# smoltcp-rs/smoltcp

Hardware: AMD Instinct MI355X
Metric: GiB/s checksummed (device-resident), batched 1500B segments, 1/2/4/8 GPU (higher is better)
Workload: dtype u8; 1 GPU; C2: 1048576 x 1500 B IPv4/UDP datagrams, fixed stride, emit (tx) + verify (rx, 1/64 single-bit corrupted); records_per_gpu=1048576, parallelism=shard x1 (no collective)

## Files before the change

### include/smolcsum_tools.h

```cpp
#ifndef SMOLCSUM_TOOLS_H
#define SMOLCSUM_TOOLS_H

#include "smolcsum.h"

#ifdef __cplusplus
extern "C" {
#endif

enum {
    SMOL_SYNTH_UDP4 = 0,
    SMOL_SYNTH_TCP4 = 1,
    SMOL_SYNTH_V6MIX = 2,
    SMOL_SYNTH_ETH_TCP4 = 3,
    SMOL_SYNTH_RANDOM = 4
};

int smol_csum_tool_synth(smol_csum_ctx_t* ctx, uint8_t* d_buf, const smol_csum_batch_t* batch,
                         int profile, uint64_t seed, void* stream);

int smol_csum_tool_corrupt(smol_csum_ctx_t* ctx, uint8_t* d_buf, const smol_csum_batch_t* batch,
                           uint32_t every, uint64_t seed, void* stream);

int smol_csum_tool_set_shape(smol_csum_ctx_t* ctx, int shape);

int smol_csum_tool_set_variant(smol_csum_ctx_t* ctx, int variant);

int smol_csum_tool_set_tile(smol_csum_ctx_t* ctx, int records);

int smol_csum_tool_set_max_blocks(smol_csum_ctx_t* ctx, uint32_t max_blocks);

int smol_csum_tool_set_xcd_remap(smol_csum_ctx_t* ctx, int on);

int smol_csum_tool_set_launch_records(smol_csum_ctx_t* ctx, uint64_t records);

int smol_csum_tool_set_fields_kernel(smol_csum_ctx_t* ctx, int kernel);

int smol_csum_tool_set_vcopy_stores(smol_csum_ctx_t* ctx, int nt);

int smol_csum_tool_stream_read(smol_csum_ctx_t* ctx, const uint8_t* d_buf, uint64_t bytes,
                               uint32_t* d_sink, void* stream);

int smol_csum_tool_field_probe(smol_csum_ctx_t* ctx, uint8_t* d_buf, uint64_t bytes, uint64_t stride,
                               uint32_t f1, uint32_t f2, void* stream);
int smol_csum_tool_field_probe_list(smol_csum_ctx_t* ctx, uint8_t* d_buf, uint64_t bytes, const uint64_t* d_addrs,
                                    const uint32_t* d_piece_first, int flags, void* stream);
int smol_csum_tool_segment_probe(smol_csum_ctx_t* ctx, uint8_t* d_buf, uint64_t bytes, const uint32_t* d_bitmap, int flags,
                                 void* stream);
int smol_csum_tool_field_scatter(smol_csum_ctx_t* ctx, uint8_t* d_buf, uint64_t bytes, const uint64_t* d_addrs,
                                 const uint16_t* d_vals, uint64_t n, int flags, void* stream);
int smol_csum_tool_auto_shape(uint32_t len, int has_desc);

int smol_csum_tool_pick(int variant, int shape, int desc_staged, int op, const smol_csum_batch_t* batch, int nhc,
                        int out[3]);
int smol_csum_tool_variant_info(int variant, int out[4]);
int smol_csum_tool_form(int variant, int op, int out[13]);
int smol_csum_tool_walk_launch(int variant, int op, int implicit, int nhc, int shape, int out[4]);

const char* smol_csum_tool_kernel_for(const smol_csum_ctx_t* ctx, int op, const smol_csum_batch_t* batch);
const char* smol_csum_tool_kernel_name(const smol_csum_ctx_t* ctx, int op, int has_desc);

uint32_t smol_csum_tool_last_launch(void);

int smol_csum_tool_variant_built(int variant);

#ifdef __cplusplus
}
#endif

#endif
```

### smoltcp_amd/_lib.py

```python
from __future__ import annotations

import ctypes
import os

_HERE = os.path.dirname(os.path.abspath(__file__))
LIB_PATH = os.environ.get("SMOLCSUM_LIB") or os.path.join(_HERE, "libsmolcsum.so")
EXP_LIB_PATH = os.path.join(_HERE, "libsmolcsum_exp.so")

SMOL_OK, SMOL_EINVAL, SMOL_ENODEV, SMOL_EHIP, SMOL_ERANGE, SMOL_ENOMEM = 0, -1, -2, -3, -4, -5
ERROR_NAMES = {
    SMOL_EINVAL: "SMOL_EINVAL",
    SMOL_ENODEV: "SMOL_ENODEV",
    SMOL_EHIP: "SMOL_EHIP",
    SMOL_ERANGE: "SMOL_ERANGE",
    SMOL_ENOMEM: "SMOL_ENOMEM",
}

ABI_SYMBOLS = [
    "smol_csum_data", "smol_csum_combine", "smol_csum_pseudo_header_v4",
    "smol_csum_pseudo_header_v6", "smol_csum_pseudo_header", "smol_csum_ctx_create",
    "smol_csum_ctx_destroy", "smol_csum_batch_data", "smol_csum_batch_emit",
    "smol_csum_batch_verify", "smol_csum_batch_copy_emit", "smol_csum_batch_emit_fields",
    "smol_csum_batch_verify_copy",
    "smol_csum_apply_fields", "smol_csum_batch_emit_frag",
    "smol_csum_batch_verify_frag", "smol_csum_batch_verify_reassemble", "smol_csum_batch_fragment_emit",
    "smol_csum_batch_nhc_udp_emit",
    "smol_csum_batch_nhc_udp_verify", "smol_csum_last_error", "smol_csum_abi_version",
]
TOOL_SYMBOLS = [
    "smol_csum_tool_synth", "smol_csum_tool_corrupt", "smol_csum_tool_set_shape",
    "smol_csum_tool_set_variant", "smol_csum_tool_set_tile",
    "smol_csum_tool_set_max_blocks", "smol_csum_tool_auto_shape", "smol_csum_tool_stream_read",
    "smol_csum_tool_set_xcd_remap", "smol_csum_tool_set_launch_records",
    "smol_csum_tool_field_probe",
    "smol_csum_tool_field_probe_list", "smol_csum_tool_segment_probe", "smol_csum_tool_field_scatter",
    "smol_csum_tool_variant_built",
    "smol_csum_tool_kernel_name", "smol_csum_tool_kernel_for", "smol_csum_tool_last_launch",
    "smol_csum_tool_pick", "smol_csum_tool_variant_info", "smol_csum_tool_form",
    "smol_csum_tool_set_fields_kernel", "smol_csum_tool_walk_launch", "smol_csum_tool_set_vcopy_stores",
]
OPTIONAL_TOOL_SYMBOLS = ("smol_csum_tool_variant_built", "smol_csum_tool_kernel_for", "smol_csum_tool_segment_probe",
                         "smol_csum_tool_pick", "smol_csum_tool_variant_info", "smol_csum_tool_form",
                         "smol_csum_tool_set_fields_kernel", "smol_csum_tool_walk_launch",
                         "smol_csum_tool_set_vcopy_stores")


class SmolError(RuntimeError):
    def __init__(self, rc: int, what: str, detail: str = ""):
        name = ERROR_NAMES.get(rc, str(rc))
        super().__init__(f"{what} failed: {name}" + (f" ({detail})" if detail else ""))
        self.rc = rc


class Caps(ctypes.Structure):

    _fields_ = [
        ("ipv4", ctypes.c_uint8),
        ("udp", ctypes.c_uint8),
        ("tcp", ctypes.c_uint8),
        ("icmpv4", ctypes.c_uint8),
        ("icmpv6", ctypes.c_uint8),
        ("reserved", ctypes.c_uint8 * 3),
    ]


class BatchC(ctypes.Structure):

    _fields_ = [
        ("desc", ctypes.c_void_p),
        ("n", ctypes.c_uint64),
        ("stride", ctypes.c_uint64),
        ("len", ctypes.c_uint32),
        ("kind", ctypes.c_uint8),
        ("flags", ctypes.c_uint8),
        ("reserved", ctypes.c_uint8 * 2),
    ]

# ... 137 lines not shown
    L.smol_csum_tool_set_variant.restype = i32
    L.smol_csum_tool_set_tile.argtypes = [vp, i32]
    L.smol_csum_tool_set_tile.restype = i32
    L.smol_csum_tool_set_max_blocks.argtypes = [vp, u32]
    L.smol_csum_tool_set_max_blocks.restype = i32
    L.smol_csum_tool_set_xcd_remap.argtypes = [vp, ctypes.c_int]
    L.smol_csum_tool_set_xcd_remap.restype = i32
    L.smol_csum_tool_set_launch_records.argtypes = [vp, u64]
    L.smol_csum_tool_set_launch_records.restype = i32
    L.smol_csum_tool_stream_read.argtypes = [vp, vp, u64, vp, vp]
    L.smol_csum_tool_stream_read.restype = i32
    L.smol_csum_tool_field_probe.argtypes = [vp, vp, u64, u64, ctypes.c_uint32, ctypes.c_uint32, vp]
    L.smol_csum_tool_field_probe.restype = i32
    L.smol_csum_tool_field_probe_list.argtypes = [vp, vp, u64, vp, vp, ctypes.c_int, vp]
    L.smol_csum_tool_field_probe_list.restype = i32
    L.smol_csum_tool_field_scatter.argtypes = [vp, vp, u64, vp, vp, u64, ctypes.c_int, vp]
    L.smol_csum_tool_field_scatter.restype = i32
    L.smol_csum_tool_auto_shape.argtypes = [u32, i32]
    L.smol_csum_tool_auto_shape.restype = i32
    L.smol_csum_tool_kernel_name.argtypes = [vp, i32, i32]
    L.smol_csum_tool_kernel_name.restype = ctypes.c_char_p
    L.smol_csum_tool_last_launch.argtypes = []
    L.smol_csum_tool_last_launch.restype = u32
    optional = {
        "smol_csum_tool_variant_built": ([i32], i32),
        "smol_csum_tool_segment_probe": ([vp, vp, u64, vp, ctypes.c_int, vp], i32),
        "smol_csum_tool_kernel_for": ([vp, i32, vp], ctypes.c_char_p),
        "smol_csum_tool_pick": ([i32, i32, i32, i32, ctypes.POINTER(BatchC), i32, ctypes.POINTER(i32)], i32),
        "smol_csum_tool_variant_info": ([i32, ctypes.POINTER(i32)], i32),
        "smol_csum_tool_form": ([i32, i32, ctypes.POINTER(i32)], i32),
        "smol_csum_tool_set_fields_kernel": ([vp, i32], i32),
        "smol_csum_tool_walk_launch": ([i32, i32, i32, i32, i32, ctypes.POINTER(i32)], i32),
        "smol_csum_tool_set_vcopy_stores": ([vp, i32], i32),
    }
    assert set(optional) == set(OPTIONAL_TOOL_SYMBOLS)
    for name in OPTIONAL_TOOL_SYMBOLS:
        if hasattr(L, name):
            f = getattr(L, name)
            f.argtypes, f.restype = optional[name]
    _LIBS[path] = L
    return L


def check(rc: int, what: str, L: ctypes.CDLL | None = None) -> None:
    if rc != SMOL_OK:
        detail = (L or lib()).smol_csum_last_error().decode(errors="replace") if rc == SMOL_EHIP else ""
        raise SmolError(rc, what, detail)
```

### smoltcp_amd/csrc/csum_api.cpp

```cpp
#include <hip/hip_runtime.h>

#include <cstdint>
#include <cstring>
#include <new>
#include <string>

#include "../../include/smolcsum.h"
#include "../../include/smolcsum_tools.h"
#include "csum_dispatch.h"

using namespace smolcsum;

struct smol_csum_ctx {
    int device;
    int num_cu;
    uint32_t max_blocks;
    int shape;
    int variant;
    uint8_t* dummy;
    int tile_records;
    bool max_blocks_set;
    int xcd_remap;
    uint64_t launch_records;
    uint64_t* stage;
    uint32_t* stage_flags;
    void* stage_stream;
    bool stage_recorded;
    hipEvent_t stage_done;
    uint32_t* sample_host;
    hipEvent_t sample_ev;
    bool sample_pending;
    int desc_staged;
    uint32_t since_probe;
    int fields_kernel;
    bool vcopy_nt;
};

namespace {
constexpr uint32_t kSample = 256;
constexpr uint32_t kReprobe = 64;
}

namespace smolcsum {

uint32_t resident_blocks(const void* kernel, uint32_t num_cu, uint32_t max_blocks) {
    if (num_cu == 0) return max_blocks;
    int per_cu = 0;
    if (hipOccupancyMaxActiveBlocksPerMultiprocessor(&per_cu, kernel, 256, 0) != hipSuccess || per_cu < 1)
        per_cu = 1;
    const uint64_t cap = (uint64_t)per_cu * num_cu;
    return (uint32_t)(cap < max_blocks ? cap : max_blocks);
}

}

namespace {

thread_local std::string g_last_error;

int hip_fail(hipError_t e, const char* what) {
    g_last_error = std::string(what) + ": " + hipGetErrorString(e);
// ... 87 lines not shown
hipError_t for_launches(const smol_csum_ctx_t* ctx, const smol_csum_batch_t* b, const KParams& p, F&& launch) {
    const uint64_t per = ctx->launch_records && ctx->launch_records < b->n ? ctx->launch_records : b->n;
    for (uint64_t i0 = 0; i0 < b->n; i0 += per) {
        KParams q = p;
        q.n = b->n - i0 < per ? b->n - i0 : per;
        if (b->desc) q.desc = b->desc + i0;
        else q.buf = p.buf + i0 * b->stride;
        const hipError_t e = launch(i0, q);
        if (e != hipSuccess) return e;
    }
    return hipSuccess;
}

PickCtx pick_ctx(const smol_csum_ctx_t* ctx) { return {ctx->variant, ctx->shape, ctx->desc_staged}; }

const char* family_kernel(int family) {
    switch (family) {
        case F_TILE: case F_STRIPE: return "csum_tile_kernel";
        case F_XWALK: return "xwalk_kernel";
        case F_DWALK: return "dwalk_kernel";
        case F_COPY: return "copy_kernel";
        case F_XCOPY: return "xcopy_kernel";
        default: return "csum_kernel";
    }
}

bool has_desc_auto(const smol_csum_ctx_t* ctx, const smol_csum_batch_t* b, const uint8_t* d_addrs) {
    return b->desc && !d_addrs && ctx->variant < 0 && !(b->flags & SMOL_BATCH_FIELD_STORES);
}

bool capturing(hipStream_t s) {
    hipStreamCaptureStatus st = hipStreamCaptureStatusNone;
    return hipStreamIsCapturing(s, &st) == hipSuccess && st != hipStreamCaptureStatusNone;
}

void update_desc_choice(smol_csum_ctx_t* ctx, hipStream_t s) {
    if (capturing(s)) return;
    if (ctx->sample_pending && hipEventQuery(ctx->sample_ev) == hipSuccess) {
        ctx->sample_pending = false;
        uint32_t n = ctx->sample_host[kSample], staged = 0;
        for (uint32_t i = 0; i < n && i < kSample; ++i) staged += ctx->sample_host[i] != 0u;
        ctx->desc_staged = n == 0 || 2 * staged >= n ? 1 : 0;
        ctx->since_probe = 0;
    }
    if (!ctx->desc_staged && !ctx->sample_pending && ++ctx->since_probe >= kReprobe) ctx->desc_staged = 1;
}

void sample_desc_choice(smol_csum_ctx_t* ctx, uint64_t n, hipStream_t s) {
    if (capturing(s) || ctx->sample_pending) return;
    const uint32_t waves = (uint32_t)((n + 7) / 8 < kSample ? (n + 7) / 8 : kSample);
    ctx->sample_host[kSample] = waves;
    if (hipMemcpyAsync(ctx->sample_host, ctx->stage_flags, waves * sizeof(uint32_t), hipMemcpyDeviceToHost, s) !=
            hipSuccess ||
        hipEventRecord(ctx->sample_ev, s) != hipSuccess) {
        (void)hipGetLastError();
        return;
    }
    ctx->sample_pending = true;
}

int run(smol_csum_ctx_t* ctx, int mode, uint8_t* d_buf, const smol_csum_batch_t* b,
        const smol_checksum_caps_t* caps, uint16_t* d_out, uint8_t* d_status, void* stream,
        const uint8_t* d_src = nullptr, const smol_csum_copy_t* d_copy = nullptr,
        const uint8_t* d_addrs = nullptr) {
    KParams p = base_params(ctx, d_buf, b, caps);
    p.src = d_src;
    p.copy = d_copy;
    if (d_addrs) p.kind = KIND_NHC_UDP;
    p.addrs = d_addrs;
    p.out16 = d_out;
    p.status = d_status;
    p.num_cu = ctx->max_blocks_set ? 0u : cu_count(ctx);
    p.xcd_remap = ctx->xcd_remap >= 0 ? (uint32_t)ctx->xcd_remap : (uint32_t)xcd_remap_auto(mode, b);
    DeviceGuard guard(ctx->device);
    if (!guard.ok) return hip_fail(hipErrorInvalidDevice, "hipSetDevice");
    const hipStream_t s = (hipStream_t)stream;
    const uint64_t per = ctx->launch_records ? ctx->launch_records : b->n;
    if (per < b->n) {
        for (uint64_t i0 = 0; i0 < b->n; i0 += per) {
            smol_csum_batch_t sub = *b;
            sub.n = b->n - i0 < per ? b->n - i0 : per;
            uint8_t* buf = d_buf;
            if (b->desc) sub.desc = b->desc + i0;
            else buf = d_buf + i0 * b->stride;
            const uint64_t keep = ctx->launch_records;
            ctx->launch_records = 0;
            const int rc = run(ctx, mode, buf, &sub, caps, d_out ? d_out + i0 : nullptr, d_status ? d_status + i0 : nullptr,
                               stream, d_src, d_copy ? d_copy + i0 : nullptr, d_addrs ? d_addrs + 32 * i0 : nullptr);
            ctx->launch_records = keep;
            if (rc != SMOL_OK) return rc;
        }
        return SMOL_OK;
    }
    const bool desc_auto = mode == MODE_EMIT && has_desc_auto(ctx, b, d_addrs);
    if (desc_auto) update_desc_choice(ctx, s);
    const Pick k = pick_kernel(pick_ctx(ctx), mode, b, p);
    if (mode == MODE_EMIT && variant_is(k.variant, V_STAGED)) {
        if (ctx->stage_recorded && ctx->stage_stream != stream) {
            hipError_t ew = hipStreamWaitEvent(s, ctx->stage_done, 0);
            if (ew != hipSuccess) return hip_fail(ew, "hipStreamWaitEvent (staged emit)");
        }
        for (uint64_t i0 = 0; i0 < b->n; i0 += kStageChunk) {
            KParams q = p;
            q.n = b->n - i0 < kStageChunk ? b->n - i0 : kStageChunk;
            if (b->desc) q.desc = b->desc + i0;
            else q.buf = d_buf + i0 * b->stride;
            if (d_status) q.status = d_status + i0;
            q.stage = ctx->stage;
            q.stage_flags = ctx->stage_flags;
            const hipError_t e = k.family == F_DWALK ? launch_dwalk(mode, k.variant, q, s) : launch_xwalk(mode, k.variant, q, s);
            if (e != hipSuccess) return hip_fail(e, "checksum kernel launch");
        }
        if (desc_auto) sample_desc_choice(ctx, b->n < kStageChunk ? b->n : kStageChunk, s);
        hipError_t er = hipEventRecord(ctx->stage_done, s);
        if (er != hipSuccess) return hip_fail(er, "hipEventRecord (staged emit)");
        ctx->stage_stream = stream;
        ctx->stage_recorded = true;
        return SMOL_OK;
    }
    hipError_t e = hipSuccess;
    switch (k.family) {
        case F_XCOPY: e = launch_xcopy(k.variant, p, s); break;
        case F_DWALK: e = launch_dwalk(mode, k.variant, p, s); break;
        case F_XWALK: e = launch_xwalk(mode, k.variant, p, s); break;
        case F_STRIPE: e = launch_stripe(mode, p, s); break;
        case F_TILE:
            e = launch_tile(mode, k.shape, find_variant(k.variant)->tile_loads, ctx->tile_records, p, ctx->max_blocks, s);
            break;
        default: e = launch_csum(mode, k.shape, k.variant, p, ctx->max_blocks, s); break;
    }
    if (e != hipSuccess) return hip_fail(e, mode == MODE_COPY ? "copy-emit kernel launch" : "checksum kernel launch");
    return SMOL_OK;
}

}

extern "C" {



int smol_csum_ctx_create(int device, smol_csum_ctx_t** out) {
    if (!out) return SMOL_EINVAL;
    *out = nullptr;
    int count = 0;
    if (hipGetDeviceCount(&count) != hipSuccess || count <= 0) {
        g_last_error = "no HIP device";
        return SMOL_ENODEV;
    }
    if (device < 0 || device >= count) return SMOL_ENODEV;
// ... 11 lines not shown
        return hip_fail(e, "hipMemset");
    }
    uint64_t* stage = nullptr;
    uint32_t* flags = nullptr;
    hipEvent_t done = nullptr;
    e = hipMalloc(&stage, kStageChunk * sizeof(uint64_t));
    if (e == hipSuccess) e = hipMalloc(&flags, (kStageChunk / 8 + 64) * sizeof(uint32_t));
    if (e == hipSuccess) e = hipEventCreateWithFlags(&done, hipEventDisableTiming);
    uint32_t* sample = nullptr;
    hipEvent_t sev = nullptr;
    if (e == hipSuccess) e = hipHostMalloc(&sample, (kSample + 1) * sizeof(uint32_t), hipHostMallocDefault);
    if (e == hipSuccess) e = hipEventCreateWithFlags(&sev, hipEventDisableTiming);
    if (e != hipSuccess) {
        (void)hipFree(dummy);
        if (stage) (void)hipFree(stage);
        if (flags) (void)hipFree(flags);
        if (sample) (void)hipHostFree(sample);
        return hip_fail(e, "context allocation");
    }
    auto* c = new (std::nothrow) smol_csum_ctx;
    if (!c) {
        (void)hipFree(dummy);
        (void)hipFree(stage);
        (void)hipFree(flags);
        (void)hipEventDestroy(done);
        (void)hipHostFree(sample);
        (void)hipEventDestroy(sev);
        return SMOL_ENOMEM;
    }
    c->dummy = dummy;
    c->stage = stage;
    c->stage_flags = flags;
    c->stage_stream = nullptr;
    c->stage_recorded = false;
    c->stage_done = done;
    c->sample_host = sample;
    c->sample_ev = sev;
    c->sample_pending = false;
    c->desc_staged = 1;
    c->since_probe = 0;
    c->fields_kernel = FK_AUTO;
    c->vcopy_nt = false;
    c->tile_records = 32;
    c->max_blocks_set = false;
    c->xcd_remap = -1;
    c->launch_records = 0;
    c->device = device;
    c->num_cu = cus;
    c->max_blocks = kNaturalGrid;
    c->shape = -1;
    c->variant = -1;
    *out = c;
    return SMOL_OK;
}

int smol_csum_ctx_destroy(smol_csum_ctx_t* ctx) {
    if (!ctx) return SMOL_OK;
    {
        DeviceGuard guard(ctx->device);
        (void)hipFree(ctx->dummy);
        (void)hipFree(ctx->stage);
        (void)hipFree(ctx->stage_flags);
        (void)hipEventDestroy(ctx->stage_done);
        if (ctx->sample_pending) (void)hipEventSynchronize(ctx->sample_ev);
        (void)hipHostFree(ctx->sample_host);
        (void)hipEventDestroy(ctx->sample_ev);
    }
// ... 186 lines not shown
    if (!ctx || !variant_built(variant)) return SMOL_EINVAL;
    ctx->variant = variant;
    return SMOL_OK;
}

int smol_csum_tool_set_tile(smol_csum_ctx_t* ctx, int records) {
    if (!ctx || (records != 32 && records != 64)) return SMOL_EINVAL;
    ctx->tile_records = records;
    return SMOL_OK;
}

int smol_csum_tool_set_max_blocks(smol_csum_ctx_t* ctx, uint32_t max_blocks) {
    if (!ctx) return SMOL_EINVAL;
    ctx->max_blocks = max_blocks ? max_blocks : kNaturalGrid;
    ctx->max_blocks_set = max_blocks != 0;
    return SMOL_OK;
}

int smol_csum_tool_set_xcd_remap(smol_csum_ctx_t* ctx, int on) {
    if (!ctx || on < -1) return SMOL_EINVAL;
    ctx->xcd_remap = on;
    return SMOL_OK;
}

int smol_csum_tool_set_launch_records(smol_csum_ctx_t* ctx, uint64_t records) {
    if (!ctx) return SMOL_EINVAL;
    ctx->launch_records = records;
    return SMOL_OK;
}

int smol_csum_tool_set_fields_kernel(smol_csum_ctx_t* ctx, int kernel) {
    if (!ctx || kernel < FK_AUTO || kernel > FK_DWALK) return SMOL_EINVAL;
    ctx->fields_kernel = kernel;
    return SMOL_OK;
}

int smol_csum_tool_set_vcopy_stores(smol_csum_ctx_t* ctx, int nt) {
    if (!ctx || (nt != 0 && nt != 1)) return SMOL_EINVAL;
    ctx->vcopy_nt = nt == 1;
    return SMOL_OK;
}

int smol_csum_tool_stream_read(smol_csum_ctx_t* ctx, const uint8_t* d_buf, uint64_t bytes,
                               uint32_t* d_sink, void* stream) {
    if (!ctx || !d_buf || !d_sink || (bytes & 15u) || ((uintptr_t)d_buf & 15u)) return SMOL_EINVAL;
    return on_device(ctx, "stream-read kernel launch", [&] {
        return launch_stream_read(d_buf, bytes, d_sink, cu_count(ctx) * 8u, (hipStream_t)stream);
    });
}

int smol_csum_tool_field_probe(smol_csum_ctx_t* ctx, uint8_t* d_buf, uint64_t bytes, uint64_t stride,
                               uint32_t f1, uint32_t f2, void* stream) {
    if (!ctx || !d_buf || (bytes & 15u) || ((uintptr_t)d_buf & 15u) || stride == 0 || f1 == ~0u) return SMOL_EINVAL;
    return on_device(ctx, "field-probe kernel launch", [&] {
        return launch_field_probe(d_buf, bytes, stride, f1, f2, cu_count(ctx) * 8u, (hipStream_t)stream);
    });
}

int smol_csum_tool_field_probe_list(smol_csum_ctx_t* ctx, uint8_t* d_buf, uint64_t bytes, const uint64_t* d_addrs,
                                    const uint32_t* d_piece_first, int flags, void* stream) {
    if (!ctx || !d_buf || !d_addrs || !d_piece_first || (bytes & 15u) || ((uintptr_t)d_buf & 15u) || (flags & ~1))
        return SMOL_EINVAL;
    return on_device(ctx, "field-probe kernel launch", [&] {
        return launch_field_probe_list(d_buf, bytes, d_addrs, d_piece_first, flags & 1, cu_count(ctx) * 8u, (hipStream_t)stream);
    });
}
// ... 124 lines not shown
```

### smoltcp_amd/csrc/csum_launch.h

```cpp
#pragma once

#include <hip/hip_runtime.h>
#include <stdint.h>

#include <atomic>

#include "../../include/smolcsum.h"
#include "csum_variants.h"

namespace smolcsum {

enum { MODE_DATA = 0, MODE_EMIT = 1, MODE_VERIFY = 2, MODE_COPY = 3 };
static_assert(MODE_DATA == kOpData && MODE_EMIT == kOpEmit && MODE_VERIFY == kOpVerify && MODE_COPY == kOpCopy, "csum_variants.h");

constexpr uint32_t KIND_NHC_UDP = 0x10;
constexpr uint32_t KIND_IPHDR_ONLY = 0x200;
__host__ __device__ __forceinline__ uint32_t desc_kind(uint32_t w) {
    return (w & 0xffu) | (((w >> 8) & SMOL_REC_IPHDR_ONLY) ? KIND_IPHDR_ONLY : 0u);
}

enum {
    CFG_G8U6 = 0,
    CFG_G16U3 = 1,
    CFG_G16U6 = 2,
// ... 163 lines not shown
inline void note_launch(uint32_t kern, uint32_t var, uint32_t g, uint32_t u) {
    g_last_launch.store(kern << 24 | (var & 0xffu) << 16 | (g & 0xffu) << 8 | (u & 0xffu),
                        std::memory_order_relaxed);
}

constexpr uint64_t kMaxGridBlocks = 0xFFFFFFull;
__host__ __device__ inline uint32_t grid_blocks(uint64_t want, uint64_t cap) {
    uint64_t b = want < cap ? want : cap;
    b = b < kMaxGridBlocks ? b : kMaxGridBlocks;
    return (uint32_t)(b ? b : 1);
}

uint32_t resident_blocks(const void* kernel, uint32_t num_cu, uint32_t max_blocks);

hipError_t launch_csum(int mode, int shape, int var, const KParams& p, uint32_t max_blocks, hipStream_t s);
template <int MODE, bool IMPLICIT>
hipError_t launch_walk(int shape, int var, const KParams& p, uint32_t max_blocks, hipStream_t s);
template <int MODE, bool IMPLICIT>
hipError_t launch_walk_nhc(int shape, int var, const KParams& p, uint32_t max_blocks, hipStream_t s);
hipError_t launch_tile(int mode, int shape, int var, int tile_records, const KParams& p, uint32_t max_blocks,
                       hipStream_t s);

hipError_t launch_stripe(int mode, const KParams& p, hipStream_t s);
hipError_t launch_dwalk(int mode, int variant, const KParams& p, hipStream_t s);
hipError_t launch_xcopy(int variant, const KParams& p, hipStream_t s);
hipError_t launch_copy_kernel(int shape, int var, const KParams& p, uint32_t max_blocks, hipStream_t s);
hipError_t launch_xwalk(int mode, int variant, const KParams& p, hipStream_t s);
constexpr uint64_t kStageChunk = 1ull << 21;
hipError_t launch_seg_pass(const KParams& p, hipStream_t s, int form = 0);
template <bool IMPLICIT>
hipError_t launch_walk_fields(int shape, const KParams& p, uint32_t max_blocks, hipStream_t s);
hipError_t launch_xwalk_fields(const KParams& p, hipStream_t s);
hipError_t launch_dwalk_fields(const KParams& p, hipStream_t s);

struct VCopyArgs {
    uint8_t* dst;
    const smol_csum_slot_t* slots;
    smol_csum_span_t* spans;
};
hipError_t launch_vcopy(int shape, bool nt, const KParams& p, const VCopyArgs& v, uint32_t max_blocks,
                        hipStream_t s);

struct SynthParams {
    uint8_t* buf;
    const smol_csum_desc_t* desc;
    uint64_t n;
    uint64_t stride;
    uint32_t len;
    uint32_t profile;
    uint64_t seed;
};
hipError_t launch_synth(const SynthParams& p, uint32_t max_blocks, hipStream_t s);
hipError_t launch_corrupt(const SynthParams& p, uint32_t every, hipStream_t s);
hipError_t launch_frag(int mode, const KParams& p, const smol_csum_frag_group_t* groups, uint64_t ngroups,
                       hipStream_t s);
struct FragCopyArgs {
    uint8_t* dst;
    const smol_csum_slot_t* slots;
    smol_csum_dgram_t* dgrams;
};
hipError_t launch_fragcopy(const KParams& p, const smol_csum_frag_group_t* groups, uint64_t ngroups,
                           const FragCopyArgs& v, hipStream_t s);
struct FragCutArgs {
    uint8_t* dst;
    const smol_csum_fragplan_t* plans;
    uint32_t frame_stride;
// ... 16 lines not shown
```

### smoltcp_amd/csrc/csum_xwalk.hip

```cpp
#include "csum_dispatch.h"
#include "csum_walk.h"

namespace smolcsum {

namespace xwalk {

constexpr int WIN_CH = 16;
constexpr int WAVES = 4;


}

template <int MODE, int R, class F>
__global__ __launch_bounds__(64 * F::WV) __attribute__((amdgpu_waves_per_eu(F::WPE > 0 ? F::WPE : 1))) void xwalk_kernel(KParams p) {
    using namespace xwalk;
    constexpr bool NOSTORE = F::NOSTORE, SEG = F::SEG, PERSIST = F::PERSIST, HALF = F::HALF, STAGE = F::STAGE;
    constexpr int NTS = F::NTS, HINT = F::HINT, WV = F::WV, STEPS = F::STEPS;
    constexpr bool EMIT = MODE == MODE_EMIT;
    constexpr int G = 64 / R;
    constexpr int NS = 16 / R;
    constexpr int GPB = WV * R;
    __shared__ u32x4 win[GPB][WIN_CH];
    __shared__ uint32_t spanbuf[GPB];
    const int wl = (int)(threadIdx.x & 63);
// ... 205 lines not shown
            if (mine && lane == 0 && r % 8 == 0) p.stage_flags[r / 8] = 1u;
        } else {
            if (wsA != ~0ull && lane < 8) seg_store(wsA + 8u * (uint32_t)lane);
            if (wsB != ~0ull && lane < 8) seg_store(wsB + 8u * (uint32_t)lane);
        }
    } else {
        if (mine)
            finish_gates<G, MODE, false, decltype(rd), 0, false, NOSTORE, (NTS & 128) != 0, false, EMIT && F::FIELDS>(
                p, g, lane == 0 ? tot : 0u, rd, winb, hd, a0, r, lane);
    }
    if (!more) break;
    wave_lds_sync();
    tw = tn;
    ++step;
    }
}

template <int MODE, int R, class F>
static void launch_xwalk_form(uint32_t blocks, const KParams& p, hipStream_t s) {
    if constexpr (F::ONLY_R != 0 && F::ONLY_R != R) {
        launch_xwalk_form<MODE, R, XPlain>(blocks, p, s);
    } else {
        if (p.len > F::MAX_LEN) return launch_xwalk_form<MODE, R, XPlain>(blocks, p, s);
        constexpr uint32_t per = (uint32_t)(F::WV / xwalk::WAVES * F::STEPS);
        uint32_t b = (blocks + per - 1) / per;
        if constexpr (F::PERSIST) {
            const uint32_t cap = resident_blocks((const void*)xwalk_kernel<MODE, R, F>, p.num_cu ? p.num_cu : 256u, b);
            b = b < cap ? b : cap;
        }
        hipLaunchKernelGGL((xwalk_kernel<MODE, R, F>), dim3(b), dim3(64 * F::WV), 0, s, p);
    }
}

hipError_t launch_xwalk_fields(const KParams& p, hipStream_t s) {
    const int R = xwalk_records(p.len);
    if (R == 0 || !p.fields) return hipErrorInvalidValue;
    const uint64_t per = (uint64_t)xwalk::WAVES * R;
    note_launch(KERN_XWALK_FIELDS, 0, 64 / R, 16 / R);
    const uint64_t span = kMaxGridBlocks * per;
    for (uint64_t i0 = 0; i0 < p.n; i0 += span) {
        KParams q = p;
        q.n = p.n - i0 < span ? p.n - i0 : span;
        q.buf = p.buf + i0 * p.stride;
        q.fields = p.fields + i0;
        const uint32_t b = grid_blocks((q.n + per - 1) / per, kMaxGridBlocks);
        switch (R) {
            case 8: launch_xwalk_form<MODE_EMIT, 8, XFields>(b, q, s); break;
            case 4: launch_xwalk_form<MODE_EMIT, 4, XFields>(b, q, s); break;
            case 2: launch_xwalk_form<MODE_EMIT, 2, XFields>(b, q, s); break;
            default: launch_xwalk_form<MODE_EMIT, 1, XFields>(b, q, s); break;
        }
        const hipError_t e = hipGetLastError();
        if (e != hipSuccess) return e;
    }
    return hipSuccess;
}

template <int R>
static bool launch_xwalk_r(int mode, int variant, uint32_t blocks, const KParams& p, hipStream_t s) {
    if (mode == MODE_EMIT) return with_xwalk_form<true>(variant, [&](auto f) { launch_xwalk_form<MODE_EMIT, R, decltype(f)>(blocks, p, s); });
    return with_xwalk_form<false>(variant, [&](auto f) { launch_xwalk_form<MODE_VERIFY, R, decltype(f)>(blocks, p, s); });
}

hipError_t launch_xwalk(int mode, int variant, const KParams& p, hipStream_t s) {
    const int R = xwalk_records(p.len);
    if (R == 0) return hipErrorInvalidValue;
    const uint64_t per = (uint64_t)xwalk::WAVES * R;
    const bool staged = mode == MODE_EMIT && variant_is(variant, V_STAGED);
    if (staged && (!p.stage || !p.stage_flags || p.n > kStageChunk)) return hipErrorInvalidValue;
    note_launch(KERN_XWALK, (uint32_t)variant, 64 / R, 16 / R);
    const uint64_t span = kMaxGridBlocks * per;
    for (uint64_t i0 = 0; i0 < p.n; i0 += span) {
        KParams q = p;
        q.n = p.n - i0 < span ? p.n - i0 : span;
        q.buf = p.buf + i0 * p.stride;
        if (p.status) q.status = p.status + i0;
        const uint32_t b = grid_blocks((q.n + per - 1) / per, kMaxGridBlocks);
        bool known;
        switch (R) {
            case 8: known = launch_xwalk_r<8>(mode, variant, b, q, s); break;
            case 4: known = launch_xwalk_r<4>(mode, variant, b, q, s); break;
            case 2: known = launch_xwalk_r<2>(mode, variant, b, q, s); break;
            default: known = launch_xwalk_r<1>(mode, variant, b, q, s); break;
        }
        if (!known) return hipErrorInvalidValue;
        hipError_t e = hipGetLastError();
        if (e != hipSuccess) return e;
        if (staged) {
// ... 9 lines not shown
```

### smoltcp_amd/engine.py

```python
from __future__ import annotations

import ctypes
from dataclasses import dataclass
from typing import Optional

import numpy as np

from . import _lib
from ._lib import NO_FIELD, BatchC, Caps, DgramC, FieldsC, FragOutC, FragPlanC, SlotC, SpanC, check, lib
from .phy import ChecksumCapabilities

KIND_RAW, KIND_IP, KIND_ETH = 0, 1, 2
REC_IPHDR_ONLY = 0x01
BATCH_FIELD_STORES = 0x80

ST_IP_OK = 0x01
ST_L4_OK = 0x02
ST_L4_PARTIAL = 0x04
ST_IP_VALID = 0x08
ST_L4_VALID = 0x10
ST_MALFORMED = 0x20
ST_UNSUPPORTED = 0x40
ST_ACCEPT = 0x80

# ... 371 lines not shown

    def field_probe(self, buf, stride: int, f1: int, f2: int = 0xFFFFFFFF, stream=None):
        nbytes = buf.numel() // 16 * 16
        check(self._L.smol_csum_tool_field_probe(self._h, buf.data_ptr(), nbytes, int(stride), int(f1), int(f2),
                                               self._stream(stream)), "smol_csum_tool_field_probe")

    def field_probe_list(self, buf, addrs, piece_first, seg64: bool = False, stream=None):
        nbytes = buf.numel() // 16 * 16
        check(self._L.smol_csum_tool_field_probe_list(self._h, buf.data_ptr(), nbytes, addrs.data_ptr(),
                                                    piece_first.data_ptr(), int(bool(seg64)),
                                                    self._stream(stream)),
              "smol_csum_tool_field_probe_list")

    def segment_probe(self, buf, bitmap, nt: bool = False, stream=None):
        nbytes = buf.numel() // 16 * 16
        check(self._L.smol_csum_tool_segment_probe(self._h, buf.data_ptr(), nbytes, bitmap.data_ptr(), int(bool(nt)),
                                                 self._stream(stream)),
              "smol_csum_tool_segment_probe")

    def field_scatter(self, buf, addrs, vals, nt: int = 0, stream=None):
        check(self._L.smol_csum_tool_field_scatter(self._h, buf.data_ptr(), buf.numel(), addrs.data_ptr(),
                                                 vals.data_ptr(), int(addrs.numel()), int(nt),
                                                 self._stream(stream)), "smol_csum_tool_field_scatter")

    def set_shape(self, shape: int):
        check(self._L.smol_csum_tool_set_shape(self._h, int(shape)), "smol_csum_tool_set_shape")

    def set_variant(self, variant: int):
        check(self._L.smol_csum_tool_set_variant(self._h, int(variant)), "smol_csum_tool_set_variant")

    def set_fields_kernel(self, kernel: int):
        check(self._L.smol_csum_tool_set_fields_kernel(self._h, int(kernel)), "smol_csum_tool_set_fields_kernel")

    def set_vcopy_stores(self, nt: bool):
        check(self._L.smol_csum_tool_set_vcopy_stores(self._h, int(bool(nt))), "smol_csum_tool_set_vcopy_stores")

    def set_tile(self, records: int):
        check(self._L.smol_csum_tool_set_tile(self._h, int(records)), "smol_csum_tool_set_tile")

    def kernel_name(self, op: str, has_desc: bool = False) -> str:
        code = {"data": 0, "emit": 1, "verify": 2, "copy_emit": 3}[op]
        return self._L.smol_csum_tool_kernel_name(self._h, code, int(bool(has_desc))).decode()

    def kernel_for(self, op: str, batch: Batch) -> str:
        code = {"data": 0, "emit": 1, "verify": 2, "copy_emit": 3}[op]
        b = batch.c()
        return self._L.smol_csum_tool_kernel_for(self._h, code, ctypes.byref(b)).decode()

    def variant_built(self, variant: int) -> bool:
        return bool(self._L.smol_csum_tool_variant_built(int(variant)))

    def last_launch(self) -> dict:
        w = int(self._L.smol_csum_tool_last_launch())
        names = {1: "csum_kernel", 2: "csum_tile_kernel", 3: "copy_kernel", 4: "csum_kernel_nhc", 5: "xwalk_kernel",
                 6: "dwalk_kernel", 7: "csum_fields_kernel", 8: "xwalk_kernel(fields)", 9: "dwalk_kernel(fields)", 10: "vcopy_kernel",
                 11: "fragcopy_kernel", 12: "fragcut_kernel"}
        if not w >> 24:
            return None
        return {"kernel": names.get(w >> 24, "?"), "variant": (w >> 16) & 0xff, "G": (w >> 8) & 0xff, "U": w & 0xff}

    def set_xcd_remap(self, on: int):
        check(self._L.smol_csum_tool_set_xcd_remap(self._h, int(on)), "smol_csum_tool_set_xcd_remap")

    def set_launch_records(self, records: int):
        check(self._L.smol_csum_tool_set_launch_records(self._h, int(records)), "smol_csum_tool_set_launch_records")

# ... 8 lines not shown
```

Measured before the change: 5571 GiB/s.

## Route large emit batches through fields kernel plus separate segment patch pass

For auto-selected xwalk emit with 1473-1921 byte records and 1M-2M records, emit is split into two steps. First the fields kernel computes checksum values into the staging scratch buffer. Then a new segment-pass kernel patches those values back into the packets with 64-byte-aligned read-modify-write nontemporal stores. The aim is to avoid the main walk writing back through the whole record, so the pass touches only the header cache lines, at the cost of an extra launch and scratch traffic. The change also adds cross-stream ordering for the shared scratch buffer and tool knobs to control the route.

```diff
diff --git a/include/smolcsum_tools.h b/include/smolcsum_tools.h
--- a/include/smolcsum_tools.h
+++ b/include/smolcsum_tools.h
@@ -37,6 +37,10 @@
 
 int smol_csum_tool_set_vcopy_stores(smol_csum_ctx_t* ctx, int nt);
 
+int smol_csum_tool_set_emit_route(smol_csum_ctx_t* ctx, int route);
+int smol_csum_tool_last_route(const smol_csum_ctx_t* ctx);
+int smol_csum_tool_set_route_chunk(smol_csum_ctx_t* ctx, uint64_t records);
+
 int smol_csum_tool_stream_read(smol_csum_ctx_t* ctx, const uint8_t* d_buf, uint64_t bytes,
                                uint32_t* d_sink, void* stream);
 
diff --git a/smoltcp_amd/_lib.py b/smoltcp_amd/_lib.py
--- a/smoltcp_amd/_lib.py
+++ b/smoltcp_amd/_lib.py
@@ -38,11 +38,13 @@
     "smol_csum_tool_kernel_name", "smol_csum_tool_kernel_for", "smol_csum_tool_last_launch",
     "smol_csum_tool_pick", "smol_csum_tool_variant_info", "smol_csum_tool_form",
     "smol_csum_tool_set_fields_kernel", "smol_csum_tool_walk_launch", "smol_csum_tool_set_vcopy_stores",
+    "smol_csum_tool_set_emit_route", "smol_csum_tool_last_route", "smol_csum_tool_set_route_chunk",
 ]
 OPTIONAL_TOOL_SYMBOLS = ("smol_csum_tool_variant_built", "smol_csum_tool_kernel_for", "smol_csum_tool_segment_probe",
                          "smol_csum_tool_pick", "smol_csum_tool_variant_info", "smol_csum_tool_form",
                          "smol_csum_tool_set_fields_kernel", "smol_csum_tool_walk_launch",
-                         "smol_csum_tool_set_vcopy_stores")
+                         "smol_csum_tool_set_vcopy_stores", "smol_csum_tool_set_emit_route",
+                         "smol_csum_tool_last_route", "smol_csum_tool_set_route_chunk")
 
 
 class SmolError(RuntimeError):
@@ -246,6 +248,9 @@
         "smol_csum_tool_set_fields_kernel": ([vp, i32], i32),
         "smol_csum_tool_walk_launch": ([i32, i32, i32, i32, i32, ctypes.POINTER(i32)], i32),
         "smol_csum_tool_set_vcopy_stores": ([vp, i32], i32),
+        "smol_csum_tool_set_emit_route": ([vp, i32], i32),
+        "smol_csum_tool_last_route": ([vp], i32),
+        "smol_csum_tool_set_route_chunk": ([vp, u64], i32),
     }
     assert set(optional) == set(OPTIONAL_TOOL_SYMBOLS)
     for name in OPTIONAL_TOOL_SYMBOLS:
diff --git a/smoltcp_amd/csrc/csum_api.cpp b/smoltcp_amd/csrc/csum_api.cpp
--- a/smoltcp_amd/csrc/csum_api.cpp
+++ b/smoltcp_amd/csrc/csum_api.cpp
@@ -25,8 +25,12 @@
     uint64_t* stage;
     uint32_t* stage_flags;
     void* stage_stream;
+    bool stage_used;
     bool stage_recorded;
     hipEvent_t stage_done;
+    int emit_route;
+    uint64_t route_chunk;
+    bool last_route;
     uint32_t* sample_host;
     hipEvent_t sample_ev;
     bool sample_pending;
@@ -180,6 +184,34 @@
 bool capturing(hipStream_t s) {
     hipStreamCaptureStatus st = hipStreamCaptureStatusNone;
     return hipStreamIsCapturing(s, &st) == hipSuccess && st != hipStreamCaptureStatusNone;
+}
+
+hipError_t order_scratch(smol_csum_ctx_t* ctx, void* stream) {
+    if (!ctx->stage_used || ctx->stage_stream == stream) return hipSuccess;
+    if (!ctx->stage_recorded) {
+        if (hipEventRecord(ctx->stage_done, (hipStream_t)ctx->stage_stream) != hipSuccess) {
+            (void)hipGetLastError();
+            ctx->stage_used = false;
+            return hipDeviceSynchronize();
+        }
+        ctx->stage_recorded = true;
+    }
+    return hipStreamWaitEvent((hipStream_t)stream, ctx->stage_done, 0);
+}
+
+constexpr uint32_t kRouteMinLen = 1473, kRouteMaxLen = 1921;
+constexpr uint64_t kRouteMinRecords = 1ull << 20, kRouteMaxRecords = 1ull << 21;
+
+bool takes_route(const smol_csum_ctx_t* ctx, int mode, const smol_csum_batch_t* b, const Pick& k, const uint8_t* d_addrs,
+                 hipStream_t s) {
+    if (mode != MODE_EMIT || ctx->emit_route == 0 || ctx->variant >= 0 || b->desc || d_addrs ||
+        (b->flags & SMOL_BATCH_FIELD_STORES) || k.family != F_XWALK ||
+        (k.variant != kXwalkEmitWT && k.variant != kXwalkEmitNt))
+        return false;
+    if (ctx->emit_route < 0 &&
+        (b->n < kRouteMinRecords || b->n > kRouteMaxRecords || b->len < kRouteMinLen || b->len > kRouteMaxLen))
+        return false;
+    return !capturing(s);
 }
 
 void update_desc_choice(smol_csum_ctx_t* ctx, hipStream_t s) {
@@ -243,11 +275,28 @@
     const bool desc_auto = mode == MODE_EMIT && has_desc_auto(ctx, b, d_addrs);
     if (desc_auto) update_desc_choice(ctx, s);
     const Pick k = pick_kernel(pick_ctx(ctx), mode, b, p);
+    if (mode == MODE_EMIT) ctx->last_route = false;
+    if (takes_route(ctx, mode, b, k, d_addrs, s)) {
+        hipError_t e = order_scratch(ctx, stream);
+        if (e != hipSuccess) return hip_fail(e, "ordering the entry buffer (emit route)");
+        ctx->stage_stream = stream;
+        ctx->stage_used = true;
+        ctx->stage_recorded = false;
+        for (uint64_t i0 = 0; i0 < b->n; i0 += ctx->route_chunk) {
+            KParams q = p;
+            q.n = b->n - i0 < ctx->route_chunk ? b->n - i0 : ctx->route_chunk;
+            q.buf = d_buf + i0 * b->stride;
+            if (d_status) q.status = d_status + i0;
+            q.fields = reinterpret_cast<smol_csum_fields_t*>(ctx->stage);
+            e = launch_xwalk_route(k.variant, q, s);
+            if (e != hipSuccess) return hip_fail(e, "checksum kernel launch (emit route)");
+        }
+        ctx->last_route = true;
+        return SMOL_OK;
+    }
     if (mode == MODE_EMIT && variant_is(k.variant, V_STAGED)) {
-        if (ctx->stage_recorded && ctx->stage_stream != stream) {
-            hipError_t ew = hipStreamWaitEvent(s, ctx->stage_done, 0);
-            if (ew != hipSuccess) return hip_fail(ew, "hipStreamWaitEvent (staged emit)");
-        }
+        const hipError_t ew = order_scratch(ctx, stream);
+        if (ew != hipSuccess) return hip_fail(ew, "hipStreamWaitEvent (staged emit)");
         for (uint64_t i0 = 0; i0 < b->n; i0 += kStageChunk) {
             KParams q = p;
             q.n = b->n - i0 < kStageChunk ? b->n - i0 : kStageChunk;
@@ -263,6 +312,7 @@
         hipError_t er = hipEventRecord(ctx->stage_done, s);
         if (er != hipSuccess) return hip_fail(er, "hipEventRecord (staged emit)");
         ctx->stage_stream = stream;
+        ctx->stage_used = true;
         ctx->stage_recorded = true;
         return SMOL_OK;
     }
@@ -340,7 +390,11 @@
     c->stage = stage;
     c->stage_flags = flags;
     c->stage_stream = nullptr;
+    c->stage_used = false;
     c->stage_recorded = false;
+    c->emit_route = -1;
+    c->route_chunk = kRouteChunk;
+    c->last_route = false;
     c->stage_done = done;
     c->sample_host = sample;
     c->sample_ev = sev;
@@ -593,6 +647,20 @@
 int smol_csum_tool_set_fields_kernel(smol_csum_ctx_t* ctx, int kernel) {
     if (!ctx || kernel < FK_AUTO || kernel > FK_DWALK) return SMOL_EINVAL;
     ctx->fields_kernel = kernel;
+    return SMOL_OK;
+}
+
+int smol_csum_tool_set_emit_route(smol_csum_ctx_t* ctx, int route) {
+    if (!ctx || route < -1 || route > 1) return SMOL_EINVAL;
+    ctx->emit_route = route;
+    return SMOL_OK;
+}
+
+int smol_csum_tool_last_route(const smol_csum_ctx_t* ctx) { return ctx ? (ctx->last_route ? 1 : 0) : SMOL_EINVAL; }
+
+int smol_csum_tool_set_route_chunk(smol_csum_ctx_t* ctx, uint64_t records) {
+    if (!ctx || records > kRouteChunk) return SMOL_EINVAL;
+    ctx->route_chunk = records ? records : kRouteChunk;
     return SMOL_OK;
 }
 
diff --git a/smoltcp_amd/csrc/csum_launch.h b/smoltcp_amd/csrc/csum_launch.h
--- a/smoltcp_amd/csrc/csum_launch.h
+++ b/smoltcp_amd/csrc/csum_launch.h
@@ -219,6 +219,9 @@
 hipError_t launch_walk_fields(int shape, const KParams& p, uint32_t max_blocks, hipStream_t s);
 hipError_t launch_xwalk_fields(const KParams& p, hipStream_t s);
 hipError_t launch_dwalk_fields(const KParams& p, hipStream_t s);
+constexpr uint64_t kRouteChunk = kStageChunk * sizeof(uint64_t) / sizeof(smol_csum_fields_t);
+hipError_t launch_xwalk_route(int variant, const KParams& p, hipStream_t s);
+hipError_t launch_seg_pass_fields(const KParams& p, hipStream_t s);
 
 struct VCopyArgs {
     uint8_t* dst;
diff --git a/smoltcp_amd/csrc/csum_segpass.hip b/smoltcp_amd/csrc/csum_segpass.hip
--- /dev/null
+++ b/smoltcp_amd/csrc/csum_segpass.hip
@@ -0,0 +1,101 @@
+#include "csum_dispatch.h"
+#include "csum_segrule.h"
+#include "csum_walk.h"
+
+namespace smolcsum {
+
+namespace segpass {
+constexpr int K = 4;
+constexpr int GROUPS = 64;
+constexpr int PER_BLOCK = K * GROUPS;
+}
+
+__global__ __launch_bounds__(256) void seg_pass_fields_kernel(KParams p) {
+    using namespace segpass;
+    const uint64_t r0 = ((uint64_t)blockIdx.x * GROUPS + (threadIdx.x >> 2)) * K;
+    const uint32_t l = threadIdx.x & 3u;
+    if (r0 >= p.n) return;
+    const uint32_t cnt = (uint32_t)(p.n - r0 < (uint64_t)K ? p.n - r0 : (uint64_t)K);
+    const uint32_t len = p.len;
+    const uint64_t stride = p.stride;
+    const uint64_t base = (uint64_t)p.buf;
+    const uint64_t total = (p.n - 1) * stride + len;
+    const uint64_t ent = (uint64_t)p.fields;
+
+    u32x4 e[K + 1];
+    e[0] = __builtin_nontemporal_load((const GMEM u32x4*)(ent + 16 * (r0 != 0 ? r0 - 1 : 0)));
+#pragma unroll
+    for (int k = 0; k < K; ++k)
+        e[k + 1] = __builtin_nontemporal_load((const GMEM u32x4*)(ent + 16 * (r0 + ((uint32_t)k < cnt ? (uint32_t)k : cnt - 1))));
+
+    SegRule d[K];
+    u32x4 xa[K], xb[K];
+#pragma unroll
+    for (int k = 0; k < K; ++k) {
+        const uint64_t r = r0 + (uint64_t)k;
+        const uint64_t a0 = base + r * stride;
+        const u32x4 en = e[k + 1], ep = e[k];
+        const uint32_t off[3] = {en.x & 0xffffu, en.x >> 16, en.y & 0xffffu};
+        const uint32_t poff[3] = {ep.x & 0xffffu, ep.x >> 16, ep.y & 0xffffu};
+        d[k] = SegRule{SEGRULE_2B, SEGRULE_2B};
+        if ((uint32_t)k < cnt)
+            d[k] = seg_rule((uint32_t)(a0 & 63u), len, stride, off, r != 0 ? segrule_field_end(poff) : SEGRULE_NO_PREV, a0 - base,
+                            total - (a0 - base));
+        xa[k] = xb[k] = u32x4{0u, 0u, 0u, 0u};
+        if (d[k].a != SEGRULE_2B) {
+            xa[k] = *(const GMEM u32x4*)(a0 + (int64_t)d[k].a + 16 * l);
+            if (d[k].b != d[k].a) xb[k] = *(const GMEM u32x4*)(a0 + (int64_t)d[k].b + 16 * l);
+        }
+    }
+
+#pragma unroll
+    for (int k = 0; k < K; ++k) {
+        if ((uint32_t)k >= cnt) break;
+        const uint64_t r = r0 + (uint64_t)k;
+        const uint64_t a0 = base + r * stride;
+        const u32x4 en = e[k + 1];
+        const uint32_t off[3] = {en.x & 0xffffu, en.x >> 16, en.y & 0xffffu};
+        const uint32_t val[3] = {en.y >> 16, en.z & 0xffffu, en.z >> 16};
+        if (p.status && l == 0) ((gu8)p.status)[r] = (uint8_t)en.w;
+        if (d[k].a == SEGRULE_2B) {
+            if (l == 0) {
+#pragma unroll
+                for (int i = 0; i < 3; ++i)
+                    if (off[i] != SEGRULE_NO_FIELD) store_be16((gu8)a0 + off[i], val[i]);
+            }
+            continue;
+        }
+        auto patch = [&](u32x4 x, uint64_t w) {
+            uint32_t xs[4] = {x.x, x.y, x.z, x.w};
+#pragma unroll
+            for (int i = 0; i < 3; ++i) {
+#pragma unroll
+                for (int j = 0; j < 2; ++j) {
+                    const uint32_t q = off[i] == SEGRULE_NO_FIELD ? 16u : (uint32_t)(a0 + off[i] + (uint32_t)j - w);
+                    const uint32_t sh = 8u * (q & 3u);
+                    const uint32_t by = (j ? val[i] : val[i] >> 8) & 0xffu;
+#pragma unroll
+                    for (uint32_t c = 0; c < 4; ++c) xs[c] = (q >> 2) == c ? (xs[c] & ~(0xffu << sh)) | (by << sh) : xs[c];
+                }
+            }
+            return u32x4{xs[0], xs[1], xs[2], xs[3]};
+        };
+        const uint64_t wa = a0 + (int64_t)d[k].a + 16 * l, wb = a0 + (int64_t)d[k].b + 16 * l;
+        const u32x4 ya = patch(xa[k], wa);
+        asm volatile("global_store_dwordx4 %0, %1, off sc0 sc1 nt" ::"v"(wa), "v"(ya) : "memory");
+        if (d[k].b != d[k].a) {
+            const u32x4 yb = patch(xb[k], wb);
+            asm volatile("global_store_dwordx4 %0, %1, off sc0 sc1 nt" ::"v"(wb), "v"(yb) : "memory");
+        }
+    }
+}
+
+hipError_t launch_seg_pass_fields(const KParams& p, hipStream_t s) {
+    if (!p.fields || p.desc || p.n == 0) return hipErrorInvalidValue;
+    const uint64_t blocks = (p.n + segpass::PER_BLOCK - 1) / segpass::PER_BLOCK;
+    if (blocks > kMaxGridBlocks) return hipErrorInvalidValue;
+    hipLaunchKernelGGL(seg_pass_fields_kernel, dim3((uint32_t)blocks), dim3(256), 0, s, p);
+    return hipGetLastError();
+}
+
+}
diff --git a/smoltcp_amd/csrc/csum_segrule.h b/smoltcp_amd/csrc/csum_segrule.h
--- /dev/null
+++ b/smoltcp_amd/csrc/csum_segrule.h
@@ -0,0 +1,45 @@
+#pragma once
+#include <cstdint>
+
+#if defined(__HIPCC__)
+#define SMOL_SEGRULE_FN __host__ __device__ inline
+#else
+#define SMOL_SEGRULE_FN inline
+#endif
+
+namespace smolcsum {
+
+constexpr uint32_t SEGRULE_NO_FIELD = 0xffffu;
+constexpr uint32_t SEGRULE_NO_PREV = ~0u;
+constexpr int32_t SEGRULE_2B = INT32_MIN;
+
+struct SegRule {
+    int32_t a, b;
+};
+
+SMOL_SEGRULE_FN uint32_t segrule_field_end(const uint32_t off[3]) {
+    uint32_t hi = 0;
+    for (int i = 0; i < 3; ++i)
+        if (off[i] != SEGRULE_NO_FIELD && off[i] + 2 > hi) hi = off[i] + 2;
+    return hi;
+}
+
+SMOL_SEGRULE_FN SegRule seg_rule(uint32_t ph, uint32_t len, uint64_t stride, const uint32_t off[3], uint32_t prev_end,
+                                 uint64_t before, uint64_t after) {
+    const SegRule two_b = {SEGRULE_2B, SEGRULE_2B};
+    uint32_t lo = SEGRULE_NO_FIELD;
+    for (int i = 0; i < 3; ++i)
+        if (off[i] < lo) lo = off[i];
+    const uint32_t hi = segrule_field_end(off);
+    if (hi == 0 || (uint64_t)hi + 64 > len) return two_b;
+    const int32_t a = (int32_t)((ph + lo) & ~63u) - (int32_t)ph;
+    const int32_t b = (int32_t)((ph + hi - 1) & ~63u) - (int32_t)ph;
+    if (b > a + 64) return two_b;
+    const bool prev_ok = stride == (uint64_t)len && before >= (uint64_t)len && prev_end != SEGRULE_NO_PREV &&
+                         (prev_end == 0 || (uint64_t)prev_end + 64 <= len);
+    if (a < 0 && !(prev_ok && (uint64_t)(-a) <= before)) return two_b;
+    if ((uint64_t)((int64_t)b + 64) > after || (uint64_t)((int64_t)b + 64) > len) return two_b;
+    return SegRule{a, b};
+}
+
+}
diff --git a/smoltcp_amd/csrc/csum_xwalk.hip b/smoltcp_amd/csrc/csum_xwalk.hip
--- a/smoltcp_amd/csrc/csum_xwalk.hip
+++ b/smoltcp_amd/csrc/csum_xwalk.hip
@@ -261,11 +261,8 @@
     }
 }
 
-hipError_t launch_xwalk_fields(const KParams& p, hipStream_t s) {
-    const int R = xwalk_records(p.len);
-    if (R == 0 || !p.fields) return hipErrorInvalidValue;
+static hipError_t launch_fields_form(int R, const KParams& p, hipStream_t s) {
     const uint64_t per = (uint64_t)xwalk::WAVES * R;
-    note_launch(KERN_XWALK_FIELDS, 0, 64 / R, 16 / R);
     const uint64_t span = kMaxGridBlocks * per;
     for (uint64_t i0 = 0; i0 < p.n; i0 += span) {
         KParams q = p;
@@ -283,6 +280,21 @@
         if (e != hipSuccess) return e;
     }
     return hipSuccess;
+}
+
+hipError_t launch_xwalk_fields(const KParams& p, hipStream_t s) {
+    const int R = xwalk_records(p.len);
+    if (R == 0 || !p.fields) return hipErrorInvalidValue;
+    note_launch(KERN_XWALK_FIELDS, 0, 64 / R, 16 / R);
+    return launch_fields_form(R, p, s);
+}
+
+hipError_t launch_xwalk_route(int variant, const KParams& p, hipStream_t s) {
+    const int R = xwalk_records(p.len);
+    if (R == 0 || !p.fields || p.desc || p.n > kRouteChunk) return hipErrorInvalidValue;
+    note_launch(KERN_XWALK, (uint32_t)variant, 64 / R, 16 / R);
+    const hipError_t e = launch_fields_form(R, p, s);
+    return e != hipSuccess ? e : launch_seg_pass_fields(p, s);
 }
 
 template <int R>
diff --git a/smoltcp_amd/engine.py b/smoltcp_amd/engine.py
--- a/smoltcp_amd/engine.py
+++ b/smoltcp_amd/engine.py
@@ -427,6 +427,15 @@
     def set_fields_kernel(self, kernel: int):
         check(self._L.smol_csum_tool_set_fields_kernel(self._h, int(kernel)), "smol_csum_tool_set_fields_kernel")
 
+    def set_emit_route(self, route: int):
+        check(self._L.smol_csum_tool_set_emit_route(self._h, int(route)), "smol_csum_tool_set_emit_route")
+
+    def last_route(self) -> bool:
+        return bool(self._L.smol_csum_tool_last_route(self._h))
+
+    def set_route_chunk(self, records: int):
+        check(self._L.smol_csum_tool_set_route_chunk(self._h, int(records)), "smol_csum_tool_set_route_chunk")
+
     def set_vcopy_stores(self, nt: bool):
         check(self._L.smol_csum_tool_set_vcopy_stores(self._h, int(bool(nt))), "smol_csum_tool_set_vcopy_stores")
 
```

Result: faster. 5726 GiB/s, median of 6 (+2.8%).
